# AIS-Bonn/vp-suite

Measured on AMD Instinct MI355X. Metric: predicted frames/sec (whole node), MovingMNIST 64x64 10->10, higher is better.
Workload: dtype bf16x3; 1 GPU; convlstm-shi (default hyper-parameters) on MovingMNIST-shaped synthetic frames 1x64x64, 10->10, random-init weights; mode=infer, per_gpu_batch=128, global_batch=128, parallelism=dp1, ranks=1, backend=single process

## Files before the change

include/vpx.h:

```cpp
#ifndef VPX_H_
#define VPX_H_

#include <stddef.h>
#include <stdint.h>

#ifdef __cplusplus
extern "C" {
#endif

#define VPX_VERSION 100

enum { VPX_OK = 0, VPX_ERR_ARG = -1, VPX_ERR_WORKSPACE = -2, VPX_ERR_LAUNCH = -3, VPX_ERR_UNSUPPORTED = -4 };

enum { VPX_GATE_IFGO = 0 ,
       VPX_GATE_IFOG = 1  };
enum { VPX_LAYOUT_NHWC = 0, VPX_LAYOUT_NCHW = 1 };
enum { VPX_PREC_F32 = 0    ,
       VPX_PREC_BF16X3 = 1 ,
       VPX_PREC_BF16 = 2    };
enum { VPX_FLAG_OUT_SPLIT = 8 ,
       VPX_FLAG_X_SPLIT = 4 ,
       VPX_FLAG_SAVE_FOR_BWD = 1 ,
       VPX_FLAG_WEIGHTS_PACKED = 2  };

// ... 9 lines not shown
    int32_t B, Cin, Ch, H, W, k;
    int32_t layer_norm;
    int32_t layout, precision, flags;
} vpx_stlstm_desc;

int vpx_version(void);
const char* vpx_last_error(void);
int vpx_set_deterministic(int on);
#define VPX_OPT_CELL2 1
#define VPX_OPT_CELL3 2
#define VPX_OPT_MFMA_SHAPE 3
#define VPX_OPT_EXPERIMENT 4
#define VPX_EXP_CELL2_FULL_TILE 4
#define VPX_EXP_CONVQ_FULL_TILE 16
#define VPX_EXP_HOIST_GEN1 32
#define VPX_EXP_ST_WGRAD_GEN1 64
#define VPX_EXP_ST_DGRAD_GEN1 128
#define VPX_EXP_ST_FWD_GEN1 256
#define VPX_EXP_C1_GEN1 512
#define VPX_EXP_C5_UNSPLIT 1024
#define VPX_EXP_C5_NO_KSPLIT 2048
#define VPX_EXP_NO_C3 4096
#define VPX_EXP_C3_NARROW 8192
#define VPX_EXP_GLUE_DGRAD_GEN1 16384
#define VPX_EXP_CELL2X 32768
#define VPX_EXP_CELL2X_COLSPLIT 65536
#define VPX_EXP_ST_LAST_FP32 (1 << 27)
#define VPX_EXP_NO_C16 (1 << 28)
#define VPX_EXP_GLUE_WGRAD_TAPGROUP (1 << 29)
#define VPX_EXP_CELL2_NO_STAGGER 1
#define VPX_EXP_CELL2_PLACEMENT 8
#define VPX_EXP_CELL2_DIAG_MASK (VPX_EXP_CELL2_NO_STAGGER | VPX_EXP_CELL2_PLACEMENT | (0xfff << 8))
#define VPX_OPT_DRY_RUN 5
int vpx_set_option(int option, int value);
int vpx_option_epoch(void);

size_t vpx_convlstm_workspace_bytes(const vpx_convlstm_desc* d);
int vpx_convlstm_takes_split_input(const vpx_convlstm_desc* d);
int vpx_convlstm_writes_split_output(const vpx_convlstm_desc* d);
size_t vpx_convlstm_reserve_bytes(const vpx_convlstm_desc* d);

int vpx_convlstm_seq_fwd(const vpx_convlstm_desc* d, const float* x, const float* h0, const float* c0,
                         const float* W, const float* bias, const float* Wci, const float* Wcf, const float* Wco,
                         float* out, float* hT, float* cT, void* reserve, size_t reserve_bytes, void* workspace,
                         size_t workspace_bytes, void* stream);

int vpx_convlstm_seq_bwd(const vpx_convlstm_desc* d, const float* x, const float* h0, const float* c0,
                         const float* W, const float* Wci, const float* Wcf, const float* Wco, const float* out,
                         const void* reserve, size_t reserve_bytes, const float* dout, const float* dhT,
                         const float* dcT, float* dx, float* dh0, float* dc0, float* dW, float* db, float* dWci,
                         float* dWcf, float* dWco, void* workspace, size_t workspace_bytes, void* stream);

enum { VPX_CL_ROUTE_FUSED = 0, VPX_CL_ROUTE_KSPLIT = 1, VPX_CL_ROUTE_HOIST = 2, VPX_CL_ROUTE_CELL3 = 3, VPX_CL_ROUTE_CELL2 = 4,
       VPX_CL_ROUTE_C3 = 5 };
typedef struct vpx_convlstm_plan_info {
    int32_t route, qform, c3nt, mw, ksplit, hh_split, hoist_convq, cell2x;
    int32_t dgrad, dgrad_qform, d_mw, dgrad_cols, wgrad, n_slices, dG_f32, gate_slices;
} vpx_convlstm_plan_info;
int vpx_convlstm_plan(const vpx_convlstm_desc* d, int x_present, int want_dx, int want_dW, vpx_convlstm_plan_info* out);

size_t vpx_stlstm_workspace_bytes(const vpx_stlstm_desc* d);
size_t vpx_stlstm_reserve_bytes(const vpx_stlstm_desc* d);
typedef struct vpx_stlstm_shadows { const void* in[5]; void* out[3]; void* dg8_out; } vpx_stlstm_shadows;
int vpx_stlstm_uses_split(const vpx_stlstm_desc* d);
int vpx_stlstm_defers_wgrad(const vpx_stlstm_desc* d);
size_t vpx_stlstm_wgrad_batch_workspace_bytes(const vpx_stlstm_desc* d);
int vpx_stlstm_wgrad_batch(const vpx_stlstm_desc* d, const void* dg8_split, const void* const* src5_split, float* dWx, float* dWh,
                           float* dWm, float* dWo, float* dWlast, void* workspace, size_t workspace_bytes, void* stream);

enum { VPX_ST_ROUTE_LN = 0, VPX_ST_ROUTE_GEN1 = 1, VPX_ST_ROUTE_C5 = 2, VPX_ST_ROUTE_C5K = 3 };
typedef struct vpx_stlstm_plan_info {
    int32_t route, o_split, nt_o, ks_g, ks_o, mw_g, mw_o, ksplit_l, last_c1;
    int32_t stw, c5, c5_ks[5], n_slices, stw_ns, dg_ksplit[5], dg_mw[5];
} vpx_stlstm_plan_info;
int vpx_stlstm_plan(const vpx_stlstm_desc* d, int all_weight_grads, vpx_stlstm_plan_info* out);

int vpx_stlstm_step_fwd(const vpx_stlstm_desc* d, const float* x, const float* h, const float* c, const float* m,
                        const float* Wx, const float* Wh, const float* Wm, const float* Wo, const float* Wlast,
                        const float* const* ln, float* h_new, float* c_new, float* m_new, float* delta_c,
                        float* delta_m, void* reserve, size_t reserve_bytes, void* workspace, size_t workspace_bytes,
                        void* stream);

int vpx_stlstm_step_bwd(const vpx_stlstm_desc* d, const float* x, const float* h, const float* c, const float* m,
                        const float* c_new, const float* m_new,
                        const float* Wx, const float* Wh, const float* Wm, const float* Wo, const float* Wlast,
                        const float* const* ln, const void* reserve, size_t reserve_bytes, const float* dh_new,
                        const float* dc_new, const float* dm_new, const float* ddelta_c, const float* ddelta_m,
                        float* dx, float* dh, float* dc, float* dm, float* dWx, float* dWh, float* dWm, float* dWo,
                        float* dWlast, float* const* dln, void* workspace, size_t workspace_bytes, void* stream);
int vpx_stlstm_step_fwd_ex(const vpx_stlstm_desc* d, const float* x, const float* h, const float* c, const float* m,
                           const float* Wx, const float* Wh, const float* Wm, const float* Wo, const float* Wlast,
                           const float* const* ln, float* h_new, float* c_new, float* m_new, float* delta_c,
// ... 271 lines not shown
```

vp-suite_amd/_lib.py:

```python
import contextlib
import ctypes
import enum
import os
import subprocess

_HERE = os.path.dirname(os.path.abspath(__file__))
LIB_PATH = os.environ.get("VPX_LIB") or os.path.join(_HERE, "libvpx_hip.so")
CSRC_DIR = os.path.join(_HERE, "csrc")

GATE_IFGO, GATE_IFOG = 0, 1
LAYOUT_NHWC, LAYOUT_NCHW = 0, 1
PREC_F32, PREC_BF16X3, PREC_BF16 = 0, 1, 2
ACT_NONE, ACT_RELU = 0, 1
RCONV_REPLICATE, RCONV_COLLAPSE = 0, 1
RCONV_EPI_PLAIN, RCONV_EPI_EVAL, RCONV_EPI_STATS = 0, 1, 2
FLAG_SAVE_FOR_BWD = 1
FLAG_WEIGHTS_PACKED = 2
FLAG_X_SPLIT = 4
FLAG_OUT_SPLIT = 8
FRAMES_U8, FRAMES_U16, FRAMES_F32 = 0, 1, 2
ACTIONS_F32, ACTIONS_F64 = 0, 1
FRAMES_AUG_ROW, FRAMES_AUG_MIN_OPS, FRAMES_AUG_MAX_OPS = 9, 16, 64
VIS_TILE_ROW = 8

OPT_CELL2 = 1
OPT_CELL3 = 2
OPT_EXPERIMENT = 4
OPT_DRY_RUN = 5
OPT_MFMA_SHAPE = 3


class Exp(enum.IntFlag):
    CELL2_FULL_TILE = 4
    CONVQ_FULL_TILE = 16
    HOIST_GEN1 = 32
    ST_WGRAD_GEN1 = 64
    ST_DGRAD_GEN1 = 128
    ST_FWD_GEN1 = 256
    C1_GEN1 = 512
    C5_UNSPLIT = 1024
    C5_NO_KSPLIT = 2048
    NO_C3 = 4096
    C3_NARROW = 8192
    GLUE_DGRAD_GEN1 = 16384
    CELL2X = 32768
    CELL2X_COLSPLIT = 65536
    ST_LAST_FP32 = 1 << 27
    NO_C16 = 1 << 28
    GLUE_WGRAD_TAPGROUP = 1 << 29
    CELL2_NO_STAGGER = 1
    CELL2_PLACEMENT = 8
    CELL2_DIAG_MASK = 1 | 8 | 0xfff << 8


class ConvLSTMDesc(ctypes.Structure):
    _fields_ = [(n, ctypes.c_int32) for n in ("B", "T", "Cin", "Ch", "H", "W", "kh", "kw", "gate_order", "layout",
                                              "precision", "flags")]


class STLSTMDesc(ctypes.Structure):
    _fields_ = [(n, ctypes.c_int32) for n in ("B", "Cin", "Ch", "H", "W", "k", "layer_norm", "layout", "precision",
# ... 39 lines not shown
CL_ROUTE_FUSED, CL_ROUTE_KSPLIT, CL_ROUTE_HOIST, CL_ROUTE_CELL3, CL_ROUTE_CELL2, CL_ROUTE_C3 = range(6)


class DensePlanInfo(ctypes.Structure):
    _fields_ = [(n, ctypes.c_int32) for n in ("split", "chunks", "chunk_len", "form", "tile_m", "tile_n", "m_tiles", "n_tiles")]


class VpxError(RuntimeError):
    pass


vp, sz, ci, ll, fl, dbl = ctypes.c_void_p, ctypes.c_size_t, ctypes.c_int, ctypes.c_longlong, ctypes.c_float, ctypes.c_double
_clstm, _stlstm, _conv, _acst, _traj = (ctypes.POINTER(D) for D in (ConvLSTMDesc, STLSTMDesc, ConvDesc, ACSTLSTMDesc, TrajGRUDesc))
_rconv = ctypes.POINTER(RConvDesc)
_int_p = ctypes.POINTER(ci)
_ws = [vp, sz, vp]
_rs_ws = [vp, sz] + _ws
_stlstm_fwd = [_stlstm] + [vp] * 4 + [vp] * 5 + [vp] + [vp] * 5 + _rs_ws
_stlstm_bwd = [_stlstm] + [vp] * 6 + [vp] * 5 + [vp] + [vp, sz] + [vp] * 5 + [vp] * 4 + [vp] * 5 + [vp] + _ws

SIGNATURES = {
    "vpx_version": (ci, []),
    "vpx_last_error": (ctypes.c_char_p, []),
    "vpx_set_deterministic": (ci, [ci]),
    "vpx_set_option": (ci, [ci, ci]),
    "vpx_option_epoch": (ci, []),
    "vpx_convlstm_workspace_bytes": (sz, [_clstm]),
    "vpx_convlstm_takes_split_input": (ci, [_clstm]),
    "vpx_convlstm_writes_split_output": (ci, [_clstm]),
    "vpx_convlstm_reserve_bytes": (sz, [_clstm]),
    "vpx_convlstm_seq_fwd": (ci, [_clstm] + [vp] * 8 + [vp] * 3 + _rs_ws),
    "vpx_convlstm_seq_bwd": (ci, [_clstm] + [vp] * 8 + [vp, sz] + [vp] * 3 + [vp] * 8 + _ws),
    "vpx_convlstm_plan": (ci, [_clstm, ci, ci, ci, vp]),
    "vpx_stlstm_workspace_bytes": (sz, [_stlstm]),
    "vpx_stlstm_reserve_bytes": (sz, [_stlstm]),
    "vpx_stlstm_uses_split": (ci, [_stlstm]),
    "vpx_stlstm_defers_wgrad": (ci, [_stlstm]),
    "vpx_stlstm_plan": (ci, [_stlstm, ci, vp]),
    "vpx_stlstm_wgrad_batch_workspace_bytes": (sz, [_stlstm]),
    "vpx_stlstm_wgrad_batch": (ci, [_stlstm, vp, vp] + [vp] * 5 + _ws),
    "vpx_stlstm_step_fwd": (ci, _stlstm_fwd),
    "vpx_stlstm_step_bwd": (ci, _stlstm_bwd),
    "vpx_stlstm_step_fwd_ex": (ci, _stlstm_fwd + [ctypes.POINTER(STLSTMShadows)]),
    "vpx_stlstm_step_bwd_ex": (ci, _stlstm_bwd + [ctypes.POINTER(STLSTMShadows)]),
    "vpx_decouple_workspace_bytes": (sz, [ci] * 4),
    "vpx_decouple_fwd": (ci, [vp] * 4 + [ci] * 5 + _ws),
    "vpx_decouple_bwd": (ci, [vp] * 7 + [ci] * 5 + _ws),
    "vpx_mse_loss_workspace_bytes": (sz, []),
    "vpx_mse_loss": (ci, [vp, vp, ll, ll, fl, vp, vp] + _ws),
    "vpx_adam_step": (ci, [vp] * 4 + [ll] + [dbl] * 5 + [ci, dbl, vp]),
    "vpx_grad_stats_workspace_bytes": (sz, []),
    "vpx_grad_stats": (ci, [vp, ll, dbl, vp] + _ws),
    "vpx_adam_step_clipped": (ci, [vp] * 4 + [ll] + [dbl] * 5 + [ci, dbl, vp, dbl, dbl, ci, vp]),
    "vpx_pixel_measures_workspace_bytes": (sz, [ll, ll]),
    "vpx_pixel_measures_fwd": (ci, [vp, vp, ll, ll, vp] + _ws),
    "vpx_pixel_measures_bwd": (ci, [vp, vp, vp, ll, ll, vp, vp]),
    "vpx_ssim_workspace_bytes": (sz, [ll, ci, ci]),
    "vpx_ssim_fwd": (ci, [vp, vp, ll] + [ci] * 4 + [vp] + _ws),
    "vpx_ssim_bwd": (ci, [vp, vp, vp, ll] + [ci] * 4 + [vp, vp]),
    "vpx_lpips_workspace_bytes": (sz, [ll, ci, ci]),
    "vpx_lpips_fwd": (ci, [vp, vp, ll] + [ci] * 3 + [vp, vp] + _ws),
    "vpx_lpips_stem_workspace_bytes": (sz, []),
    "vpx_lpips_stem_fwd": (ci, [vp, vp, ll, ll, ci, ci, vp, vp, vp] + _ws),
    "vpx_lpips_maxpool_fwd": (ci, [vp, vp, ll] + [ci] * 3 + [vp]),
    "vpx_lpips_head_workspace_bytes": (sz, [ll, ll]),
    "vpx_lpips_head_fwd": (ci, [vp, vp, vp, ll, ll, ci, vp] + _ws),
# ... 168 lines not shown
```

vp-suite_amd/csrc/convlstm_fwd_api.hip:

```cpp
#include "vpx_host.h"
using namespace vpx;

static int c3_nt(const vpx_convlstm_desc* d, const ConvLSTMLayout& L) {
    if (!L.v2 || !cell2_q_applicable(d) || d->precision != VPX_PREC_BF16X3 || (d->flags & VPX_FLAG_SAVE_FOR_BWD) || exp_on(VPX_EXP_NO_C3)) return 0;
    if ((d->Cin & 7) || (d->Ch & 15)) return 0;
    const long long mt = (long long)d->B * ((d->H + 15) / 16) * ((d->W + 15) / 16);
    constexpr int C3_MAX = 256;
    if (mt * L.n_tiles > C3_MAX) return 0;
    return exp_on(VPX_EXP_C3_NARROW) ? 2 : 4;
}

enum class Route {
    FUSED,
    KSPLIT,
    HOIST,
    CELL3,
    CELL2,
    C3,
};
struct RouteChoice { Route route; int qform, c3nt; };
static RouteChoice convlstm_route(const vpx_convlstm_desc* d, const ConvLSTMLayout& L, bool x_present) {
    if (L.v3) return {Route::CELL3, 0, 0};
    if (L.v2) { const int nt = c3_nt(d, L); return {nt ? Route::C3 : Route::CELL2, cell2_q_applicable(d) ? 1 : 0, nt}; }
    if (L.hoist && x_present) return {Route::HOIST, 0, 0};
    return {L.split ? Route::KSPLIT : Route::FUSED, 0, 0};
}
static bool on_cell2(const RouteChoice& r) { return r.route == Route::CELL2 || r.route == Route::C3; }
static bool on_ksplit(const RouteChoice& r) { return r.route == Route::KSPLIT || r.route == Route::HOIST; }
static bool inference_nhwc(const vpx_convlstm_desc* d) { return d->layout == VPX_LAYOUT_NHWC && !(d->flags & VPX_FLAG_SAVE_FOR_BWD); }

static size_t cell2_wpk_bytes(const vpx_convlstm_desc* d, const ConvLSTMLayout& L) {
    const int S = (d->Cin + d->Ch) / 16;
    const size_t a = cell2_packed_bytes(L.n_tiles, 3 * S), b = cell2_packed_bytes_q(L.n_tiles, S);
// ... 77 lines not shown
}

extern "C" {
size_t vpx_convlstm_reserve_bytes(const vpx_convlstm_desc* d) {
    ConvLSTMLayout L;
    if (check_convlstm_desc(d) != VPX_OK || convlstm_layout(d, L) != VPX_OK) return 0;
    return convlstm_reserve(d, L, nullptr).bytes;
}
int vpx_convlstm_takes_split_input(const vpx_convlstm_desc* d) { return split_format(d, true); }
int vpx_convlstm_writes_split_output(const vpx_convlstm_desc* d) { return split_format(d, false); }

size_t vpx_convlstm_workspace_bytes(const vpx_convlstm_desc* d) {
    ConvLSTMLayout L;
    if (check_convlstm_desc(d) != VPX_OK || convlstm_layout(d, L) != VPX_OK) return 0;
    const RouteChoice r = convlstm_route(d, L, true);
    ConvQProblem hq; CarveMeasure m; FwdSlots s{};
    carve_fwd(m, d, L, r, route_hoists_on_convq(d, r, hq) ? &hq : nullptr, s);
    const size_t bwd = (d->flags & VPX_FLAG_SAVE_FOR_BWD) ? convlstm_bwd_workspace_bytes(d, L) : 0;
    return (m.off > bwd ? m.off : bwd) + 256;
}
}

struct FwdCtx {
    const vpx_convlstm_desc* d; const ConvLSTMLayout* L; RouteChoice r;
    const float *x, *h0, *c0, *W, *bias, *wci, *wcf, *wco;
    float *out, *hT, *cT;
    FwdSlots ws;
    ConvLSTMReserve res;
    int gp[4]; hipStream_t stream; size_t HW;
    bool save, wp, x_split, out_split;
    bool hoist_q; ConvQProblem hq;
};

static int stage_in_nchw(FwdCtx& c) {
    const FwdSlots& s = c.ws;
    const int B = c.d->B, T = c.d->T, Cin = c.d->Cin, Ch = c.d->Ch, H = c.d->H, Wd = c.d->W;
    if (c.x) { VPX_CHECK_HIP(launch_nchw_to_nhwc(c.x, s.bx, B * T, Cin, H, Wd, c.stream)); c.x = s.bx; }
    if (c.h0) { VPX_CHECK_HIP(launch_nchw_to_nhwc(c.h0, s.bh0, B, Ch, H, Wd, c.stream)); c.h0 = s.bh0; }
    if (c.c0) { VPX_CHECK_HIP(launch_nchw_to_nhwc(c.c0, s.bc0, B, Ch, H, Wd, c.stream)); c.c0 = s.bc0; }
    const float** peep[3] = {&c.wci, &c.wcf, &c.wco};
    for (int i = 0; i < 3 && c.wci; ++i) { VPX_CHECK_HIP(launch_nchw_to_nhwc(*peep[i], s.bpeep[i], 1, Ch, H, Wd, c.stream)); *peep[i] = s.bpeep[i]; }
    c.out = s.bout; c.hT = c.hT ? s.bhT : nullptr; c.cT = c.cT ? s.bcT : nullptr;
    return VPX_OK;
}
static ConvSeg h_prev(const FwdCtx& c, int t) {
    const size_t n = c.HW * c.d->Ch;
    return t == 0 ? ConvSeg{c.h0, (long long)n, c.d->Ch, 0} : ConvSeg{c.out + (size_t)(t - 1) * n, (long long)(c.d->T * n), c.d->Ch, 0};
}

static int gen1_pack(const FwdCtx& c) {
    const vpx_convlstm_desc* d = c.d; const ConvLSTMLayout& L = *c.L;
    PackDesc pd{};
    const long long ld_o = (long long)(d->Cin + d->Ch) * L.taps;
    pd.seg[0] = PackSeg{c.W, ld_o, L.taps, 0, d->Cin};
    pd.seg[1] = PackSeg{c.W, ld_o, L.taps, d->Cin, d->Ch};
    pd.prec = d->precision; pd.taps = L.taps;
    if (on_ksplit(c.r)) {
        memcpy(pd.stage, L.s_stage, sizeof(ConvStage) * L.s_nstage);
        pd.nstage = L.s_nstage; pd.chunks_total = L.s_chunks;
        fill_plain_pack(pd, 4 * d->Ch, 0, L.s_ng);
    } else {
        memcpy(pd.stage, L.stage, sizeof(ConvStage) * L.nstage);
        pd.nstage = L.nstage; pd.chunks_total = L.chunks_total; pd.qpc = L.qpc; pd.n_tiles = L.n_tiles; pd.NG = 4;
        for (int g = 0; g < 4; ++g) { pd.rowbase[0][g] = pd.rowbase[1][g] = c.gp[g] * d->Ch; pd.goff[g] = 0; }
        pd.tile_stride = 32; pd.nch = d->Ch;
    }
// ... 133 lines not shown
    if (combo & 2) for (int s = 0; s < Ch / 16; ++s) pk.stage_col[pk.S++] = Cin + 16 * s;
    pk.chunks_total = cell2_qchunks(pk.S);
    if (c.wp) return VPX_OK;
    if (!c.r.c3nt) { VPX_CHECK_HIP(launch_cell2_pack(pk, cell2_pack_of(c, combo), c.stream)); return VPX_OK; }
    C5Job j{};
    C5PackRange pr[2];
    const long long so = (long long)(Cin + Ch) * 9;
    if (combo & 1) { j.r_n[j.nrange] = Cin; pr[j.nrange] = C5PackRange{c.W, so, 9, 0, {gp[0] * Ch, gp[1] * Ch, gp[2] * Ch, gp[3] * Ch}}; ++j.nrange; }
    if (combo & 2) { j.r_n[j.nrange] = Ch; pr[j.nrange] = C5PackRange{c.W, so, 9, Cin, {gp[0] * Ch, gp[1] * Ch, gp[2] * Ch, gp[3] * Ch}}; ++j.nrange; }
    j.Co = Ch; j.wpk = cell2_pack_of(c, combo);
    return c5_prepare_job(j, c.r.c3nt, pr, 4, 0, false, c.stream, 0, 3);
}
static int cell2_pack(FwdCtx& c) {
    const vpx_convlstm_desc* d = c.d; const int Cin = d->Cin, Ch = d->Ch;
    const int combo0 = (c.x ? 1 : 0) | (c.h0 ? 2 : 0), combo1 = (c.x ? 1 : 0) | 2;
    Cell2Pack pk{};
    pk.w = c.W; pk.Ch = Ch; pk.Ct = Cin + Ch; pk.n_tiles = c.L->n_tiles;
    memcpy(pk.gate_pos, c.gp, sizeof(c.gp));
    if (!c.r.qform) {
        pk.chunks_total = 3 * ((Cin + Ch) / 16);
        for (int s = 0; s < (Cin + Ch) / 16; ++s) pk.stage_col[s] = 16 * s;
        if (!c.wp) VPX_CHECK_HIP(launch_cell2_pack(pk, c.ws.wpk2, c.stream));
    } else {
        int rc;
        if (!(d->T < 2 && combo0 != combo1) && (rc = cell2_pack_combo(c, pk, combo1)) != VPX_OK) return rc;
        if (combo0 != combo1 && combo0 != 0 && (rc = cell2_pack_combo(c, pk, combo0)) != VPX_OK) return rc;
    }
    if (c.save) { c.ws.x_sp = c.res.x_sp; c.ws.h0_sp = c.res.h0_sp; }
    if (c.x && c.x_split) c.ws.x_sp = const_cast<char*>(reinterpret_cast<const char*>(c.x));
    else if (c.x) VPX_CHECK_HIP(launch_split_convert(c.x, c.ws.x_sp, (long long)d->B * d->T * (long long)c.HW, Cin, c.stream));
    if (c.h0) VPX_CHECK_HIP(launch_split_convert(c.h0, c.ws.h0_sp, (long long)d->B * (long long)c.HW, Ch, c.stream));
    return VPX_OK;
}
static int cell2_step(const FwdCtx& c, int t, ConvLSTMStepArgs ea) {
    const vpx_convlstm_desc* d = c.d; const int T = d->T, Cin = d->Cin, Ch = d->Ch; const size_t HW = c.HW;
    Cell2Plan P2{};
    P2.B = d->B; P2.H = d->H; P2.W = d->W; P2.tiles_x = (d->W + 15) / 16; P2.tiles_y = (d->H + 31) / 32; P2.n_tiles = c.L->n_tiles;
    P2.chunks_total = 3 * ((Cin + Ch) / 16); P2.wpk = c.ws.wpk2;
    P2.qform = c.r.qform; P2.plain = d->precision == VPX_PREC_BF16 ? 1 : 0;
    const long long hsp_bs = c.out_split ? (long long)((size_t)T * HW * Ch * 4) : (long long)(HW * Ch * 4);
    if (c.out_split) { ea.h_out = (t == T - 1) ? c.hT : nullptr; ea.h_bstride = (long long)(HW * Ch); }
    const char* hprev_sp = (t == 0) ? (c.h0 ? c.ws.h0_sp : nullptr) : cell2_h_slot(c, t - 1);
    P2.seg[0] = Cell2Seg{c.x ? c.ws.x_sp + (size_t)t * HW * Cin * 4 : nullptr, (long long)((size_t)T * HW * Cin * 4), Cin, 0};
    P2.seg[1] = Cell2Seg{hprev_sp, (t == 0) ? (long long)(HW * Ch * 4) : hsp_bs, Ch, 0};
    P2.nx = c.x ? Cin / 16 : 0; P2.nh = hprev_sp ? Ch / 16 : 0; P2.hs_off = Cin / 16;
    if (c.r.qform) {
        P2.chunks_total = cell2_qchunks(P2.nx + P2.nh);
        P2.wpk = cell2_pack_of(c, (P2.nx ? 1 : 0) | (P2.nh ? 2 : 0));
    }
    char* const hsp_t = (t + 1 < T || c.out_split) ? cell2_h_slot(c, t) : nullptr;
    if (c.r.route == Route::CELL2) { VPX_CHECK_HIP(launch_cell2(P2, ea, hsp_t, hsp_bs, c.stream)); return VPX_OK; }
    C5Plan cp{};
    cp.B = P2.B; cp.H = P2.H; cp.W = P2.W; cp.ks = 3;
    cp.src[0] = C5Src{P2.seg[0].sp, P2.seg[0].bstride, Cin * 4, 0};
    cp.src[1] = C5Src{P2.seg[1].sp, P2.seg[1].bstride, Ch * 4, 0};
    C5Job& j = cp.job[cp.njobs++] = C5Job{};
    if (P2.nx) { j.r_src[j.nrange] = 0; j.r_n[j.nrange] = Cin; ++j.nrange; }
    if (P2.nh) { j.r_src[j.nrange] = 1; j.r_n[j.nrange] = Ch; ++j.nrange; }
    j.epi = 3; j.Co = Ch; j.Ch = Ch; j.wpk = P2.wpk;
    j.e_in0 = ea.c_in; j.e_in1 = ea.wci; j.e_in2 = ea.wcf; j.e_in3 = ea.wco; j.bias = ea.bias;
    for (int g = 0; g < 4; ++g) j.gate_pos[g] = ea.gate_pos[g];
    j.e_out[0] = ea.h_out; j.e_out[1] = ea.c_out; j.h_bstride = ea.h_bstride;
    j.e_sp = hsp_t; j.sp_bstride = hsp_bs;
    const int rcj = c5_prepare_job(j, c.r.c3nt, nullptr, 4, 0, true, c.stream, 0, 3);
    if (rcj) return rcj;
    VPX_CHECK_HIP(launch_c5(cp, c.r.c3nt, c.stream));
    return VPX_OK;
}

static ConvLSTMStepArgs step_args(const FwdCtx& c, int t) {
    const size_t n = c.L->n_state;
    ConvLSTMStepArgs ea{};
    ea.bias = c.bias; ea.Ch = c.d->Ch;
    memcpy(ea.gate_pos, c.gp, sizeof(c.gp));
    if (c.save) {
        ea.c_in = (t == 0) ? c.c0 : c.res.cs + (size_t)(t - 1) * n;
        ea.c_out = c.res.cs + (size_t)t * n; ea.gates = c.res.gates + (size_t)t * n * 4;
    } else {
        ea.c_in = (t == 0) ? c.c0 : c.ws.c_scratch;
        ea.c_out = (t == c.d->T - 1 && c.cT) ? c.cT : c.ws.c_scratch;
    }
    ea.wci = c.wci; ea.wcf = c.wcf; ea.wco = c.wco;
    ea.h_out = c.out + (size_t)t * c.HW * c.d->Ch;
    ea.h_bstride = (long long)((size_t)c.d->T * c.HW * c.d->Ch);
    return ea;
}
extern "C" int vpx_convlstm_seq_fwd(const vpx_convlstm_desc* d, const float* x, const float* h0, const float* c0,
                                    const float* W, const float* bias, const float* Wci, const float* Wcf, const float* Wco,
                                    float* out, float* hT, float* cT, void* reserve, size_t reserve_bytes, void* workspace,
                                    size_t workspace_bytes, void* stream_) {
    int rc = check_convlstm_desc(d);
    if (rc != VPX_OK) return rc;
    ConvLSTMLayout L;
    if ((rc = convlstm_layout(d, L)) != VPX_OK) return rc;
    if (!W || !out) { set_error("vpx_convlstm_seq_fwd: W and out must not be NULL"); return VPX_ERR_ARG; }
    if ((Wci || Wcf || Wco) && !(Wci && Wcf && Wco)) { set_error("vpx_convlstm_seq_fwd: peephole tensors must be given together"); return VPX_ERR_ARG; }
    FwdCtx c{};
    c.d = d; c.L = &L; c.stream = (hipStream_t)stream_; c.HW = (size_t)d->H * d->W;
    c.x = x; c.h0 = h0; c.c0 = c0; c.W = W; c.bias = bias; c.wci = Wci; c.wcf = Wcf; c.wco = Wco;
    c.out = out; c.hT = hT; c.cT = cT;
    c.save = (d->flags & VPX_FLAG_SAVE_FOR_BWD) != 0; c.x_split = (d->flags & VPX_FLAG_X_SPLIT) != 0;
    c.wp = (d->flags & VPX_FLAG_WEIGHTS_PACKED) != 0; c.out_split = (d->flags & VPX_FLAG_OUT_SPLIT) != 0;
    if (c.out_split && !vpx_convlstm_writes_split_output(d)) {
        set_error("vpx_convlstm_seq_fwd: VPX_FLAG_OUT_SPLIT given, but this descriptor's forward writes fp32 only (vpx_convlstm_writes_split_output)"); return VPX_ERR_ARG;
    }
    if (c.x_split && !vpx_convlstm_takes_split_input(d)) {
        set_error("vpx_convlstm_seq_fwd: VPX_FLAG_X_SPLIT given, but this descriptor's forward takes fp32 input (vpx_convlstm_takes_split_input)"); return VPX_ERR_ARG;
    }
    c.res = convlstm_reserve(d, L, reserve);
    if (c.save && (!reserve || reserve_bytes < c.res.bytes)) { set_error("vpx_convlstm_seq_fwd: reserve too small (%zu < %zu)", reserve_bytes, c.res.bytes); return VPX_ERR_WORKSPACE; }
    if (!workspace || workspace_bytes < vpx_convlstm_workspace_bytes(d)) {
        set_error("vpx_convlstm_seq_fwd: workspace too small (%zu < %zu)", workspace_bytes, vpx_convlstm_workspace_bytes(d)); return VPX_ERR_WORKSPACE;
    }
    c.r = convlstm_route(d, L, x != nullptr);
    c.hoist_q = route_hoists_on_convq(d, c.r, c.hq);
    Carver ws(workspace, workspace_bytes);
    carve_fwd(ws, d, L, c.r, c.hoist_q ? &c.hq : nullptr, c.ws);
    VPX_CHECK_CARVE(ws, "vpx_convlstm_seq_fwd");
    if (d->layout == VPX_LAYOUT_NCHW && (rc = stage_in_nchw(c)) != VPX_OK) return rc;
    gate_positions(d->gate_order, c.gp);
    switch (c.r.route) {
        case Route::FUSED: case Route::KSPLIT: case Route::HOIST: rc = gen1_pack(c); break;
        case Route::CELL3: rc = cell3_pack(c); break;
        case Route::CELL2: case Route::C3: rc = cell2_pack(c); break;
    }
    if (rc != VPX_OK) return rc;
    if ((c.r.route == Route::HOIST || c.r.route == Route::CELL3) && c.x && (rc = hoisted_projection(c)) != VPX_OK) return rc;
    for (int t = 0; t < d->T; ++t) {
        const ConvLSTMStepArgs ea = step_args(c, t);
        switch (c.r.route) {
            case Route::FUSED: rc = fused_step(c, t, ea); break;
            case Route::KSPLIT: rc = ksplit_step(c, t, ea); break;
            case Route::HOIST: rc = hoist_step(c, t, ea); break;
            case Route::CELL3: rc = cell3_step(c, t, ea); break;
            case Route::CELL2: case Route::C3: rc = cell2_step(c, t, ea); break;
        }
        if (rc != VPX_OK) return rc;
    }
    const int B = d->B, T = d->T, Ch = d->Ch;
    if (c.cT && c.save)
        VPX_CHECK_HIP(vpx_memcpy_async(c.cT, c.res.cs + (size_t)(T - 1) * L.n_state, L.n_state * sizeof(float), hipMemcpyDeviceToDevice, c.stream));
    if (c.hT && !c.out_split)
        VPX_CHECK_HIP(vpx_memcpy2d_async(c.hT, c.HW * Ch * sizeof(float), c.out + (size_t)(T - 1) * c.HW * Ch,
                                       (size_t)T * c.HW * Ch * sizeof(float), c.HW * Ch * sizeof(float), B, hipMemcpyDeviceToDevice, c.stream));
    if (d->layout == VPX_LAYOUT_NCHW) {
        VPX_CHECK_HIP(launch_nhwc_to_nchw(c.out, out, B * T, Ch, d->H, d->W, c.stream));
        if (hT) VPX_CHECK_HIP(launch_nhwc_to_nchw(c.hT, hT, B, Ch, d->H, d->W, c.stream));
        if (cT) VPX_CHECK_HIP(launch_nhwc_to_nchw(c.cT, cT, B, Ch, d->H, d->W, c.stream));
    }
    return VPX_OK;
}

extern "C" int vpx_convlstm_plan(const vpx_convlstm_desc* d, int x_present, int want_dx, int want_dW, vpx_convlstm_plan_info* out) {
    int rc = check_convlstm_desc(d);
    if (rc != VPX_OK) return rc;
    if (!out) { set_error("vpx_convlstm_plan: out is NULL"); return VPX_ERR_ARG; }
    ConvLSTMLayout L;
    if ((rc = convlstm_layout(d, L)) != VPX_OK) return rc;
    const RouteChoice r = convlstm_route(d, L, x_present != 0);
    ConvQProblem hq;
    *out = vpx_convlstm_plan_info{};
    out->route = (int)r.route; out->qform = r.qform; out->c3nt = r.c3nt;
    out->mw = r.route == Route::FUSED ? L.mw : 0;
    out->ksplit = r.route == Route::KSPLIT ? L.split : 0;
    out->hh_split = r.route == Route::HOIST ? L.hh_split : 0;
    out->hoist_convq = x_present && route_hoists_on_convq(d, r, hq) ? 1 : 0;
    out->cell2x = r.route == Route::CELL2 && cell2_step_on_x(r.qform) ? 1 : 0;
    if (d->flags & VPX_FLAG_SAVE_FOR_BWD) convlstm_bwd_plan(d, L, x_present != 0, want_dx != 0, want_dW != 0, out);
    return VPX_OK;
}
```

vp-suite_amd/csrc/vpx_api.hip:

```cpp
#include <stdarg.h>
#include <stdio.h>
#include <string.h>

#include "vpx_host.h"

namespace vpx {

static thread_local char g_err[512] = "";

void set_error(const char* fmt, ...) {
    va_list ap;
    va_start(ap, fmt);
    vsnprintf(g_err, sizeof(g_err), fmt, ap);
    va_end(ap);
}

static thread_local Carver* g_carver = nullptr;
static thread_local char g_ws_violation[256] = "";

Carver::Carver(void* workspace, size_t bytes)
    : base((char*)workspace), off((256 - ((uintptr_t)workspace & 255)) & 255), cap(bytes), nslot(0), over(false), prev(g_carver) {
    if (off > cap) over = true;
    if (!prev) c5_drop_pending_packs();
    g_carver = this;
    g_ws_violation[0] = 0;
}
Carver::~Carver() { g_carver = prev; }

const char* ws_violation() { return g_ws_violation; }
void ws_violation_clear() { g_ws_violation[0] = 0; }

bool ws_write_ok(const void* dst_, size_t bytes, const char* what) {
    const char* dst = (const char*)dst_;
    for (const Carver* c = g_carver; c; c = c->prev) {
        if (dst < c->base || dst >= c->base + c->cap) continue;
        const char* end = c->base + c->cap;
        size_t room = (size_t)(end - dst);
        for (int i = 0; i < c->nslot; ++i)
            if (dst >= c->slot[i].p && dst < c->slot[i].p + c->slot[i].n) { room = (size_t)(c->slot[i].p + c->slot[i].n - dst); break; }
        if (bytes <= room) return true;
        snprintf(g_ws_violation, sizeof(g_ws_violation), "%s: %zu bytes do not fit the %zu bytes carved for them (workspace sizing rule and launch disagree)",
                 what, bytes, room);
        return false;
    }
    return true;
}

int g_dry_run = 0;
int g_deterministic = 0;
int g_cell3_mode = 1;
int g_cell2_mode = 1;
int g_experiment = 0;
int g_mfma_shape = 1;

}

using namespace vpx;

extern "C" {

int vpx_version(void) { return VPX_VERSION; }
static int g_option_epoch = 0;
int vpx_option_epoch(void) { return g_option_epoch; }
int vpx_set_deterministic(int on) { const int prev = vpx::g_deterministic; vpx::g_deterministic = on ? 1 : 0; ++g_option_epoch; return prev; }
const char* vpx_last_error(void) { return g_err; }
int vpx_set_option(int option, int value) {
    ++g_option_epoch;
    if (option == VPX_OPT_CELL2) {
        const int prev = g_cell2_mode;
        vpx::g_cell2_mode = value < 0 ? 0 : (value > 2 ? 2 : value);
        return prev;
    }
    if (option == VPX_OPT_EXPERIMENT) {
        const int prev = vpx::g_experiment;
        vpx::g_experiment = value;
        return prev;
    }
    if (option == VPX_OPT_MFMA_SHAPE) {
        const int prev = g_mfma_shape;
        vpx::g_mfma_shape = value ? 1 : 0;
        return prev;
    }
    if (option == VPX_OPT_DRY_RUN) {
        const int prev = vpx::g_dry_run;
        vpx::g_dry_run = value ? 1 : 0;
        return prev;
    }
    if (option == VPX_OPT_CELL3) {
        const int prev = g_cell3_mode;
        vpx::g_cell3_mode = value ? 1 : 0;
        return prev;
    }
    set_error("vpx_set_option: unknown option %d", option);
    return VPX_ERR_ARG;
}

int vpx_nchw_to_nhwc(const float* src, float* dst, int N, int C, int H, int W, void* stream) {
    if (!src || !dst || N < 1 || C < 1 || H < 1 || W < 1) { set_error("vpx_nchw_to_nhwc: bad argument"); return VPX_ERR_ARG; }
    VPX_CHECK_HIP(launch_nchw_to_nhwc(src, dst, N, C, H, W, (hipStream_t)stream));
    return VPX_OK;
}
int vpx_nhwc_to_nchw(const float* src, float* dst, int N, int C, int H, int W, void* stream) {
    if (!src || !dst || N < 1 || C < 1 || H < 1 || W < 1) { set_error("vpx_nhwc_to_nchw: bad argument"); return VPX_ERR_ARG; }
    VPX_CHECK_HIP(launch_nhwc_to_nchw(src, dst, N, C, H, W, (hipStream_t)stream));
    return VPX_OK;
}

int vpx_split_convert(const float* x, void* x_split, long long n_pixels, int C, void* stream) {
    if (!x || !x_split || n_pixels < 0 || C < 8 || (C & 7)) { set_error("vpx_split_convert: NULL tensor or channel count %d not a multiple of 8", C); return VPX_ERR_ARG; }
    VPX_CHECK_HIP(launch_split_convert(x, x_split, n_pixels, C, (hipStream_t)stream));
    return VPX_OK;
}

}
```

vp-suite_amd/csrc/vpx_internal.h:

```cpp
#pragma once
#include <stdlib.h>
#include <hip/hip_runtime.h>
#include <stdint.h>
#include <stddef.h>

#include "../../include/vpx.h"

namespace vpx {

constexpr int TILE_H = 8;
constexpr int TILE_W = 16;
constexpr int NTHREADS = 256;
constexpr int NT = 128;
constexpr int MAX_NG = 4;
constexpr int CS_MAX = 64;
constexpr int MAX_SEG = 3;
constexpr int MAX_STAGE = 32;

struct ConvSeg {
    const float* ptr;
    long long bstride;
    int C;
    int ld;
    int split, _p;
// ... 116 lines not shown
    float* c_out;
    const float* wci;
    const float* wcf;
    const float* wco;
    float* h_out;
    long long h_bstride;
    float* gates;
};
hipError_t launch_convlstm_step_f32(const ConvPlan& plan, const ConvLSTMStepArgs& ea, int n_tiles, hipStream_t s);
struct Cell2Seg { const char* sp; long long bstride; int C; int _pad; };
struct Cell2Plan {
    int B, H, W, tiles_x, tiles_y, n_tiles, nx, nh, hs_off, chunks_total, grid_m, _p;
    int qform, _q;
    int plain;
    int n_groups, gpt;
    Cell2Seg seg[2];
    const char* wpk;
};
static inline int cell2_qchunks(int S) { return (9 * S + 1) / 2; }
struct Cell2Pack {
    const float* w;
    int Ch, Ct, n_tiles, chunks_total;
    int qform, S;
    int gate_pos[4];
    int stage_col[MAX_STAGE];
};
hipError_t launch_split_convert(const float* src, void* dst, long long npix, int C, hipStream_t s);
hipError_t launch_cell2_pack(const Cell2Pack& pk, void* dst, hipStream_t s);
size_t cell2_packed_bytes(int n_tiles, int chunks_total);
size_t cell2_packed_bytes_q(int n_tiles, int S);
extern int g_experiment;
static inline bool exp_on(int bit) { return (g_experiment & bit) != 0; }
extern int g_mfma_shape;
hipError_t launch_cell2(const Cell2Plan& plan, const ConvLSTMStepArgs& ea, void* h_sp, long long h_sp_bstride, hipStream_t s);
hipError_t launch_cell2x(const Cell2Plan& plan, const ConvLSTMStepArgs& ea, void* h_sp, long long h_sp_bstride, hipStream_t s);
static inline bool cell2x_selected() { return exp_on(VPX_EXP_CELL2X); }
static inline bool cell2_step_on_x(int qform) { return qform && cell2x_selected(); }
bool c16_applicable(const ::vpx_conv_desc* d);
size_t c16_wpk_bytes(const ::vpx_conv_desc* d);
int c16_forward(const ::vpx_conv_desc* d, const char* x_split, long long x_bstride, long long x_tstride, int x_nT, const float* w,
                const float* bias, float* y, char* y_split, char* wpk, bool packed, hipStream_t s);
static inline int conv2_tiles(int Co) { return ((Co + 31) / 32 + 3) / 4; }
static inline int conv2_gpt(int Co) { const int g = (Co + 31) / 32, t = (g + 3) / 4; return (g + t - 1) / t; }
struct Conv2Pack {
    const float* w; long long s_oc, s_ic;
    int Co, col0, n_tiles, gpt, chunks_total, flip;
    int qform, _p;
};
struct Conv2Args {
    int B, H, W, C, Co, split, accumulate, qform;
    const char* src_sp; long long src_bstride;
    const char* wpk; const float* bias;
    float* out0; long long bstride0; int ld0, _p0;
    float* out1; long long bstride1; int ld1, _p1;
};
hipError_t launch_conv2_pack(const Conv2Pack& pk, void* dst, hipStream_t s);
hipError_t launch_conv2(const Conv2Args& c, hipStream_t s);

struct CQSeg {
    const char* sp;
    long long bstride, tstride; int nT, _p0;
    int rowpitch, colpitch;
    int org;
    int Hs, Ws;
    int nstage, c0;
    int _p1;
// ... 349 lines not shown
```

Baseline: 54250 frames/s.

## Split ConvLSTM sequence batch into two chains on separate streams

```diff
diff --git a/include/vpx.h b/include/vpx.h
--- a/include/vpx.h
+++ b/include/vpx.h
@@ -65,6 +65,7 @@
 #define VPX_EXP_CELL2_PLACEMENT 8
 #define VPX_EXP_CELL2_DIAG_MASK (VPX_EXP_CELL2_NO_STAGGER | VPX_EXP_CELL2_PLACEMENT | (0xfff << 8))
 #define VPX_OPT_DRY_RUN 5
+#define VPX_OPT_SEQ_CHAINS 6
 int vpx_set_option(int option, int value);
 int vpx_option_epoch(void);
 
@@ -91,6 +92,7 @@
     int32_t dgrad, dgrad_qform, d_mw, dgrad_cols, wgrad, n_slices, dG_f32, gate_slices;
 } vpx_convlstm_plan_info;
 int vpx_convlstm_plan(const vpx_convlstm_desc* d, int x_present, int want_dx, int want_dW, vpx_convlstm_plan_info* out);
+int vpx_convlstm_seq_chains(const vpx_convlstm_desc* d, int x_present, void* stream);
 
 size_t vpx_stlstm_workspace_bytes(const vpx_stlstm_desc* d);
 size_t vpx_stlstm_reserve_bytes(const vpx_stlstm_desc* d);
diff --git a/vp-suite_amd/_lib.py b/vp-suite_amd/_lib.py
--- a/vp-suite_amd/_lib.py
+++ b/vp-suite_amd/_lib.py
@@ -27,6 +27,7 @@
 OPT_CELL3 = 2
 OPT_EXPERIMENT = 4
 OPT_DRY_RUN = 5
+OPT_SEQ_CHAINS = 6
 OPT_MFMA_SHAPE = 3
 
 
@@ -132,6 +133,7 @@
     "vpx_convlstm_seq_fwd": (ci, [_clstm] + [vp] * 8 + [vp] * 3 + _rs_ws),
     "vpx_convlstm_seq_bwd": (ci, [_clstm] + [vp] * 8 + [vp, sz] + [vp] * 3 + [vp] * 8 + _ws),
     "vpx_convlstm_plan": (ci, [_clstm, ci, ci, ci, vp]),
+    "vpx_convlstm_seq_chains": (ci, [_clstm, ci, vp]),
     "vpx_stlstm_workspace_bytes": (sz, [_stlstm]),
     "vpx_stlstm_reserve_bytes": (sz, [_stlstm]),
     "vpx_stlstm_uses_split": (ci, [_stlstm]),
diff --git a/vp-suite_amd/csrc/convlstm_fwd_api.hip b/vp-suite_amd/csrc/convlstm_fwd_api.hip
--- a/vp-suite_amd/csrc/convlstm_fwd_api.hip
+++ b/vp-suite_amd/csrc/convlstm_fwd_api.hip
@@ -1,4 +1,6 @@
 #include "vpx_host.h"
+
+#include <mutex>
 using namespace vpx;
 
 static int c3_nt(const vpx_convlstm_desc* d, const ConvLSTMLayout& L) {
@@ -142,6 +144,8 @@
     bool hoist_q; ConvQProblem hq;
 };
 
+struct Chain { int b0, B; hipStream_t stream; };
+
 static int stage_in_nchw(FwdCtx& c) {
     const FwdSlots& s = c.ws;
     const int B = c.d->B, T = c.d->T, Cin = c.d->Cin, Ch = c.d->Ch, H = c.d->H, Wd = c.d->W;
@@ -341,24 +345,25 @@
     if (c.h0) VPX_CHECK_HIP(launch_split_convert(c.h0, c.ws.h0_sp, (long long)d->B * (long long)c.HW, Ch, c.stream));
     return VPX_OK;
 }
-static int cell2_step(const FwdCtx& c, int t, ConvLSTMStepArgs ea) {
-    const vpx_convlstm_desc* d = c.d; const int T = d->T, Cin = d->Cin, Ch = d->Ch; const size_t HW = c.HW;
+static int cell2_step(const FwdCtx& c, int t, ConvLSTMStepArgs ea, const Chain& ch) {
+    const vpx_convlstm_desc* d = c.d; const int T = d->T, Cin = d->Cin, Ch = d->Ch; const size_t HW = c.HW, b0 = (size_t)ch.b0;
     Cell2Plan P2{};
-    P2.B = d->B; P2.H = d->H; P2.W = d->W; P2.tiles_x = (d->W + 15) / 16; P2.tiles_y = (d->H + 31) / 32; P2.n_tiles = c.L->n_tiles;
+    P2.B = ch.B; P2.H = d->H; P2.W = d->W; P2.tiles_x = (d->W + 15) / 16; P2.tiles_y = (d->H + 31) / 32; P2.n_tiles = c.L->n_tiles;
     P2.chunks_total = 3 * ((Cin + Ch) / 16); P2.wpk = c.ws.wpk2;
     P2.qform = c.r.qform; P2.plain = d->precision == VPX_PREC_BF16 ? 1 : 0;
     const long long hsp_bs = c.out_split ? (long long)((size_t)T * HW * Ch * 4) : (long long)(HW * Ch * 4);
-    if (c.out_split) { ea.h_out = (t == T - 1) ? c.hT : nullptr; ea.h_bstride = (long long)(HW * Ch); }
+    if (c.out_split) { ea.h_out = (t == T - 1 && c.hT) ? c.hT + b0 * HW * Ch : nullptr; ea.h_bstride = (long long)(HW * Ch); }
     const char* hprev_sp = (t == 0) ? (c.h0 ? c.ws.h0_sp : nullptr) : cell2_h_slot(c, t - 1);
     P2.seg[0] = Cell2Seg{c.x ? c.ws.x_sp + (size_t)t * HW * Cin * 4 : nullptr, (long long)((size_t)T * HW * Cin * 4), Cin, 0};
     P2.seg[1] = Cell2Seg{hprev_sp, (t == 0) ? (long long)(HW * Ch * 4) : hsp_bs, Ch, 0};
+    for (Cell2Seg& sg : P2.seg) if (sg.sp) sg.sp += b0 * (size_t)sg.bstride;
     P2.nx = c.x ? Cin / 16 : 0; P2.nh = hprev_sp ? Ch / 16 : 0; P2.hs_off = Cin / 16;
     if (c.r.qform) {
         P2.chunks_total = cell2_qchunks(P2.nx + P2.nh);
         P2.wpk = cell2_pack_of(c, (P2.nx ? 1 : 0) | (P2.nh ? 2 : 0));
     }
-    char* const hsp_t = (t + 1 < T || c.out_split) ? cell2_h_slot(c, t) : nullptr;
-    if (c.r.route == Route::CELL2) { VPX_CHECK_HIP(launch_cell2(P2, ea, hsp_t, hsp_bs, c.stream)); return VPX_OK; }
+    char* const hsp_t = (t + 1 < T || c.out_split) ? cell2_h_slot(c, t) + b0 * (size_t)hsp_bs : nullptr;
+    if (c.r.route == Route::CELL2) { VPX_CHECK_HIP(launch_cell2(P2, ea, hsp_t, hsp_bs, ch.stream)); return VPX_OK; }
     C5Plan cp{};
     cp.B = P2.B; cp.H = P2.H; cp.W = P2.W; cp.ks = 3;
     cp.src[0] = C5Src{P2.seg[0].sp, P2.seg[0].bstride, Cin * 4, 0};
@@ -371,28 +376,66 @@
     for (int g = 0; g < 4; ++g) j.gate_pos[g] = ea.gate_pos[g];
     j.e_out[0] = ea.h_out; j.e_out[1] = ea.c_out; j.h_bstride = ea.h_bstride;
     j.e_sp = hsp_t; j.sp_bstride = hsp_bs;
-    const int rcj = c5_prepare_job(j, c.r.c3nt, nullptr, 4, 0, true, c.stream, 0, 3);
+    const int rcj = c5_prepare_job(j, c.r.c3nt, nullptr, 4, 0, true, ch.stream, 0, 3);
     if (rcj) return rcj;
-    VPX_CHECK_HIP(launch_c5(cp, c.r.c3nt, c.stream));
-    return VPX_OK;
-}
-
-static ConvLSTMStepArgs step_args(const FwdCtx& c, int t) {
-    const size_t n = c.L->n_state;
+    VPX_CHECK_HIP(launch_c5(cp, c.r.c3nt, ch.stream));
+    return VPX_OK;
+}
+
+static ConvLSTMStepArgs step_args(const FwdCtx& c, int t, const Chain& ch) {
+    const size_t n = c.L->n_state, off = (size_t)ch.b0 * c.HW * c.d->Ch;
     ConvLSTMStepArgs ea{};
     ea.bias = c.bias; ea.Ch = c.d->Ch;
     memcpy(ea.gate_pos, c.gp, sizeof(c.gp));
     if (c.save) {
         ea.c_in = (t == 0) ? c.c0 : c.res.cs + (size_t)(t - 1) * n;
-        ea.c_out = c.res.cs + (size_t)t * n; ea.gates = c.res.gates + (size_t)t * n * 4;
+        ea.c_out = c.res.cs + (size_t)t * n + off; ea.gates = c.res.gates + (size_t)t * n * 4 + 4 * off;
     } else {
         ea.c_in = (t == 0) ? c.c0 : c.ws.c_scratch;
-        ea.c_out = (t == c.d->T - 1 && c.cT) ? c.cT : c.ws.c_scratch;
-    }
+        ea.c_out = ((t == c.d->T - 1 && c.cT) ? c.cT : c.ws.c_scratch) + off;
+    }
+    if (ea.c_in) ea.c_in += off;
     ea.wci = c.wci; ea.wcf = c.wcf; ea.wco = c.wco;
-    ea.h_out = c.out + (size_t)t * c.HW * c.d->Ch;
     ea.h_bstride = (long long)((size_t)c.d->T * c.HW * c.d->Ch);
+    ea.h_out = c.out + (size_t)t * c.HW * c.d->Ch + (size_t)ch.b0 * (size_t)ea.h_bstride;
     return ea;
+}
+
+constexpr int SEQ_CHAINS_MIN_B = 8;
+static int seq_chains(const vpx_convlstm_desc* d, const RouteChoice& r, hipStream_t stream) {
+    if (!on_cell2(r) || g_seq_chains == 0 || d->B < (g_seq_chains == 2 ? 2 : SEQ_CHAINS_MIN_B)) return 1;
+    if (g_dry_run) return 2;
+    hipStreamCaptureStatus st = hipStreamCaptureStatusNone;
+    if (hipStreamIsCapturing(stream, &st) != hipSuccess) { (void)hipGetLastError(); return 1; }
+    return st == hipStreamCaptureStatusNone ? 2 : 1;
+}
+struct SeqSide { hipStream_t stream; hipEvent_t fork, join; bool made; };
+static std::mutex g_side_mutex;
+static SeqSide g_side[64];
+static int seq_side(SeqSide*& out) {
+    int dev = 0;
+    VPX_CHECK_HIP(hipGetDevice(&dev));
+    if (dev < 0 || dev >= 64) { set_error("vpx_convlstm_seq_fwd: device %d beyond the side-stream table", dev); return VPX_ERR_UNSUPPORTED; }
+    std::lock_guard<std::mutex> lock(g_side_mutex);
+    SeqSide& sd = g_side[dev];
+    if (!sd.made) {
+        VPX_CHECK_HIP(hipStreamCreateWithFlags(&sd.stream, hipStreamNonBlocking));
+        VPX_CHECK_HIP(hipEventCreateWithFlags(&sd.fork, hipEventDisableTiming));
+        VPX_CHECK_HIP(hipEventCreateWithFlags(&sd.join, hipEventDisableTiming));
+        sd.made = true;
+    }
+    out = &sd;
+    return VPX_OK;
+}
+static hipError_t seq_order(hipEvent_t ev, hipStream_t from, hipStream_t to) {
+    std::lock_guard<std::mutex> lock(g_side_mutex);
+    const hipError_t e = hipEventRecord(ev, from);
+    return e != hipSuccess ? e : hipStreamWaitEvent(to, ev, 0);
+}
+extern "C" int vpx_convlstm_seq_chains(const vpx_convlstm_desc* d, int x_present, void* stream) {
+    ConvLSTMLayout L;
+    if (check_convlstm_desc(d) != VPX_OK || convlstm_layout(d, L) != VPX_OK) return 0;
+    return seq_chains(d, convlstm_route(d, L, x_present != 0), (hipStream_t)stream);
 }
 extern "C" int vpx_convlstm_seq_fwd(const vpx_convlstm_desc* d, const float* x, const float* h0, const float* c0,
                                     const float* W, const float* bias, const float* Wci, const float* Wcf, const float* Wco,
@@ -435,17 +478,36 @@
     }
     if (rc != VPX_OK) return rc;
     if ((c.r.route == Route::HOIST || c.r.route == Route::CELL3) && c.x && (rc = hoisted_projection(c)) != VPX_OK) return rc;
-    for (int t = 0; t < d->T; ++t) {
-        const ConvLSTMStepArgs ea = step_args(c, t);
-        switch (c.r.route) {
-            case Route::FUSED: rc = fused_step(c, t, ea); break;
-            case Route::KSPLIT: rc = ksplit_step(c, t, ea); break;
-            case Route::HOIST: rc = hoist_step(c, t, ea); break;
-            case Route::CELL3: rc = cell3_step(c, t, ea); break;
-            case Route::CELL2: case Route::C3: rc = cell2_step(c, t, ea); break;
+    Chain chain[2] = {{0, d->B, c.stream}, {0, 0, c.stream}};
+    const int nchain = seq_chains(d, c.r, c.stream);
+    SeqSide* side = nullptr;
+    if (nchain == 2) {
+        chain[0].B = (d->B + 1) / 2;
+        chain[1].b0 = chain[0].B; chain[1].B = d->B - chain[0].B;
+        if (!g_dry_run) {
+            if ((rc = seq_side(side)) != VPX_OK) return rc;
+            VPX_CHECK_HIP(c5_flush_packs(c.stream));
+            VPX_CHECK_HIP(seq_order(side->fork, c.stream, side->stream));
+            chain[1].stream = side->stream;
         }
-        if (rc != VPX_OK) return rc;
-    }
+    }
+    for (int t = 0; t < d->T && rc == VPX_OK; ++t)
+        for (int k = 0; k < nchain && rc == VPX_OK; ++k) {
+            const Chain& ch = chain[k];
+            const ConvLSTMStepArgs ea = step_args(c, t, ch);
+            switch (c.r.route) {
+                case Route::FUSED: rc = fused_step(c, t, ea); break;
+                case Route::KSPLIT: rc = ksplit_step(c, t, ea); break;
+                case Route::HOIST: rc = hoist_step(c, t, ea); break;
+                case Route::CELL3: rc = cell3_step(c, t, ea); break;
+                case Route::CELL2: case Route::C3: rc = cell2_step(c, t, ea, ch); break;
+            }
+        }
+    if (side) {
+        const hipError_t ej = seq_order(side->join, side->stream, c.stream);
+        if (rc == VPX_OK) VPX_CHECK_HIP(ej);
+    }
+    if (rc != VPX_OK) return rc;
     const int B = d->B, T = d->T, Ch = d->Ch;
     if (c.cT && c.save)
         VPX_CHECK_HIP(vpx_memcpy_async(c.cT, c.res.cs + (size_t)(T - 1) * L.n_state, L.n_state * sizeof(float), hipMemcpyDeviceToDevice, c.stream));
diff --git a/vp-suite_amd/csrc/vpx_api.hip b/vp-suite_amd/csrc/vpx_api.hip
--- a/vp-suite_amd/csrc/vpx_api.hip
+++ b/vp-suite_amd/csrc/vpx_api.hip
@@ -51,6 +51,7 @@
 int g_cell3_mode = 1;
 int g_cell2_mode = 1;
 int g_experiment = 0;
+int g_seq_chains = 1;
 int g_mfma_shape = 1;
 
 }
@@ -86,6 +87,11 @@
         vpx::g_dry_run = value ? 1 : 0;
         return prev;
     }
+    if (option == VPX_OPT_SEQ_CHAINS) {
+        const int prev = g_seq_chains;
+        vpx::g_seq_chains = value < 0 ? 0 : (value > 2 ? 2 : value);
+        return prev;
+    }
     if (option == VPX_OPT_CELL3) {
         const int prev = g_cell3_mode;
         vpx::g_cell3_mode = value ? 1 : 0;
diff --git a/vp-suite_amd/csrc/vpx_internal.h b/vp-suite_amd/csrc/vpx_internal.h
--- a/vp-suite_amd/csrc/vpx_internal.h
+++ b/vp-suite_amd/csrc/vpx_internal.h
@@ -172,6 +172,7 @@
 extern int g_experiment;
 static inline bool exp_on(int bit) { return (g_experiment & bit) != 0; }
 extern int g_mfma_shape;
+extern int g_seq_chains;
 hipError_t launch_cell2(const Cell2Plan& plan, const ConvLSTMStepArgs& ea, void* h_sp, long long h_sp_bstride, hipStream_t s);
 hipError_t launch_cell2x(const Cell2Plan& plan, const ConvLSTMStepArgs& ea, void* h_sp, long long h_sp_bstride, hipStream_t s);
 static inline bool cell2x_selected() { return exp_on(VPX_EXP_CELL2X); }
```

Result: faster. 54990 frames/s (median of 6 runs) (+1.4%).
